# LIS-TU-Berlin/SVN-ICP

Hardware: AMD Instinct MI355X
Metric: scan-pair registrations/sec at N particles x M source pts, 1/2/4/8 GPU (higher is better)
Workload: dtype f64; 1 GPU; C3: 128 particles SVN-ICP, 131072-pt source vs 262144-pt target, K=100, I=20, max_dist=1.0, lr=1.0, SVNFullGrad=False, correspondence=fast, early stop off; synthetic 64-beam scans (seed 20250718); particles=128, target_points=262144, knn_count=100, parallelism=single GPU

## Files before the change

### include/svnicp_hip.h

```cpp
#ifndef SVNICP_HIP_H
#define SVNICP_HIP_H

#include <stdint.h>

#ifdef __cplusplus
extern "C" {
#endif

#define SVNICP_ABI_VERSION 1

typedef struct svnicp_ctx svnicp_ctx;

#define SVNICP_ALIGN_SUCCESS 1
#define SVNICP_NO_OPTIMIZER 2

typedef enum {
  SVNICP_OK = 0,
  SVNICP_ERR_INVALID = -1,
  SVNICP_ERR_HIP = -2,
  SVNICP_ERR_NO_DEVICE = -3,
  SVNICP_ERR_NOMEM = -4
} svnicp_status;

#define SVNICP_MODE_SVN 0
// ... 143 lines not shown
int svnicp_get_mode_labels(svnicp_ctx *ctx, int32_t *outP);

int svnicp_set_shard(svnicp_ctx *ctx, int p_lo, int p_hi);
int svnicp_set_row_shard(svnicp_ctx *ctx, int row_rank, int row_world, int64_t total_source_points);
void *svnicp_rank_sums_devptr(svnicp_ctx *ctx);
int svnicp_align_begin(svnicp_ctx *ctx);
int svnicp_stage_candidates(svnicp_ctx *ctx, int64_t b_lo, int64_t b_hi);
int svnicp_build_candidate_table(svnicp_ctx *ctx);
int svnicp_iter_accumulate(svnicp_ctx *ctx, int iteration);
int svnicp_iter_update(svnicp_ctx *ctx, int iteration);
int svnicp_finish(svnicp_ctx *ctx);
int svnicp_stopped(svnicp_ctx *ctx);
void *svnicp_candidates_devptr(svnicp_ctx *ctx);
void *svnicp_sums_devptr(svnicp_ctx *ctx);
void *svnicp_total_pose_devptr(svnicp_ctx *ctx);
#define SVNICP_NSUMS 22

typedef struct svnicp_map svnicp_map;
int svnicp_map_create(int device, double voxel_size, double max_range, int max_points, int64_t capacity_voxels,
                      svnicp_map **out);
void svnicp_map_destroy(svnicp_map *map);
const char *svnicp_map_last_error(const svnicp_map *map);
int svnicp_map_clear(svnicp_map *map);
int svnicp_map_size(svnicp_map *map, int64_t *voxels);
int svnicp_map_add_cloud(svnicp_map *map, const float *xyz, int64_t n, int mem_kind, const double R_rowmajor[9],
                         const double t[3]);
int svnicp_map_skipped_points(svnicp_map *map, int64_t *out);
int svnicp_map_table_info(svnicp_map *map, int64_t *capacity_slots, int64_t *tombstones, int64_t *rebuilds);
int svnicp_map_query(svnicp_map *map, const double center[3], double max_range, int64_t *count_out);
void *svnicp_map_points_devptr(svnicp_map *map);
// ... 92 lines not shown
```

### svn-icp_amd/binding.py

```python
from __future__ import annotations

import ctypes as C
import os
import re

_HERE = os.path.dirname(os.path.abspath(__file__))
_ROOT = os.path.dirname(_HERE)
_LIB_PATH = os.path.join(_HERE, "libsvnicp_hip.so")
_HEADER = os.path.join(_ROOT, "include", "svnicp_hip.h")


class SvnIcpError(RuntimeError):
    pass


class Params(C.Structure):
    _fields_ = [("struct_size", C.c_int32), ("mode", C.c_int32), ("iterations", C.c_int32),
                ("knn_count", C.c_int32), ("lr", C.c_double), ("max_dist", C.c_double),
                ("convergence_threshold", C.c_double), ("check_early_stop", C.c_int32),
                ("svn_full_grad", C.c_int32), ("optimizer", C.c_int32), ("record_trace", C.c_int32)]


class SegParamsStruct(C.Structure):
    _fields_ = [("struct_size", C.c_int32), ("n_scan", C.c_int32), ("horizon_scan", C.c_int32), ("ground_scan_ind", C.c_int32),
# ... 158 lines not shown
    L.svnicp_rank_sums_devptr.argtypes = [vp]
    L.svnicp_rank_sums_devptr.restype = vp
    L.svnicp_align_begin.argtypes = [vp]
    L.svnicp_stage_candidates.argtypes = [vp, C.c_int64, C.c_int64]
    L.svnicp_build_candidate_table.argtypes = [vp]
    L.svnicp_iter_accumulate.argtypes = [vp, C.c_int]
    L.svnicp_iter_update.argtypes = [vp, C.c_int]
    L.svnicp_finish.argtypes = [vp]
    L.svnicp_stopped.argtypes = [vp]
    L.svnicp_candidates_devptr.argtypes = [vp]
    L.svnicp_candidates_devptr.restype = vp
    L.svnicp_sums_devptr.argtypes = [vp]
    L.svnicp_sums_devptr.restype = vp
    L.svnicp_total_pose_devptr.argtypes = [vp]
    L.svnicp_total_pose_devptr.restype = vp
    L.svnicp_set_minibatch.argtypes = [vp, C.c_int, C.c_uint64]
    L.svnicp_set_minibatch_indices.argtypes = [vp, vp, C.c_int, C.c_int, C.c_int]
    L.svnicp_get_minibatch_indices.argtypes = [vp, ip]
    L.svnicp_get_minibatch_candidates.argtypes = [vp, ip]
    L.svnicp_get_minibatch_rows.argtypes = [vp, C.POINTER(C.c_int64)]
    L.svnicp_set_residual.argtypes = [vp, C.c_int, C.c_double, C.c_int]
    L.svnicp_set_target_normals.argtypes = [vp, vp, C.c_int64, C.c_int]
    L.svnicp_get_target_normals.argtypes = [vp, dp]
    L.svnicp_get_plane_stats.argtypes = [vp, dp, C.POINTER(C.c_int64)]
    L.svnicp_evaluate.argtypes = [vp, dp, dp, C.c_double, C.POINTER(EvalStruct)]
    for name in ("svnicp_eval_index_devptr", "svnicp_eval_dist2_devptr"):
        getattr(L, name).argtypes = [vp]
        getattr(L, name).restype = vp
    L.svnicp_get_eval_pairs.argtypes = [vp, ip, dp]
    L.svnicp_eval_information.argtypes = [vp, C.c_int, C.c_double, C.c_double, C.POINTER(InformationStruct)]
# ... 15 lines not shown
```

### svn-icp_amd/csrc/api.hip

```cpp
#include "../../include/svnicp_hip.h"

#include <cmath>
#include <algorithm>
#include <cstdio>
#include <cstdlib>
#include <cstring>
#include <string>
#include <vector>

#include "device_buffer.hpp"
#include "information_solve.hpp"
#include "kernels.hpp"
#include "stage_a_host.hpp"
#include "stage_b_host.hpp"

using namespace svnicp;
using namespace svnicp_host;

namespace {

struct CloudState {
  DevBuf<double> src, tgt;
  bool src_set = false, tgt_set = false;
};
// ... 400 lines not shown
  else if (k == "wgpcu") { int x = 0, y = 0; ok = sscanf(v.c_str(), "%d,%d", &x, &y) == 2 && x >= 0 && x <= 64 && y >= 0 && y <= 16; if (ok) { t.wgpcu_search = x; t.wgpcu_accum = y; } }
  else if (k == "tp") ok = num(0, 1 << 16, &t.tp);
  else if (k == "debug") ok = num(0, 1, &t.debug);
  else if (k == "scan_split") ok = num(0, 16, &t.scan_split);
  else if (k == "group_stride") ok = num(0, 1 << 30, &t.group_stride);
  else if (k == "accum_min_steps") ok = num(0, 1 << 20, &t.accum_min_steps);
  else if (k == "brute_qb") { ok = num(0, 6, &t.brute_qb); }
  else if (k == "single") { if (v == "fused") t.single_fused = 1; else if (v == "split") t.single_fused = 0; else ok = false; }
  else if (k == "chain") { if (v == "auto") { t.small_chain = 1; t.persistent = 0; } else if (v == "persistent") { t.small_chain = 1; t.persistent = 1; }
                           else if (v == "general") { t.small_chain = 0; t.persistent = 0; } else ok = false; }
  else if (k == "median") { if (v == "auto") t.median_inline = -1; else if (v == "stream") t.median_inline = 0; else if (v == "inline") t.median_inline = 1; else ok = false; }
  else if (k == "sort") { if (v == "joint") t.sort_joint = 1; else if (v == "separate") t.sort_joint = 0; else ok = false; }
  else if (k == "sort_kernel") { if (v == "radix") t.sort_merge = 0; else if (v == "merge") t.sort_merge = 1; else ok = false; }
  else if (k == "table") { if (v == "select") t.table_select = 1; else if (v == "gather") t.table_select = 0; else ok = false; }
  else if (k == "correspondence") { if (v == "fast") t.full_corr = 0; else if (v == "full") t.full_corr = 1; else ok = false; }
  else return fail(c, SVNICP_ERR_INVALID, "svnicp_set_option: unknown option '" + k + "'");
  if (!ok) return fail(c, SVNICP_ERR_INVALID, "svnicp_set_option: bad value '" + v + "' for option '" + k + "'");
  c->run.have_candidates = false;
  c->sa.held = TargetLayout::None;
  if (c->run.began) c->st.step = plan_step(registration_facts(c, c->pl.on), c->tune, c->sb.plan);
  return SVNICP_OK;
}

int svnicp_set_shard(svnicp_ctx* c, int p_lo, int p_hi) {
  CTX_CHECK(c);
  if (!c->run.particles_set || p_lo < 0 || p_hi > c->P || p_lo > p_hi)
    return fail(c, SVNICP_ERR_INVALID, "svnicp_set_shard: need 0 <= p_lo <= p_hi <= P after svnicp_set_particles");
  c->shard.p_lo = p_lo; c->shard.p_hi = p_hi; c->shard.set = true;
  return SVNICP_OK;
}
// ... 227 lines not shown
  }
  u.eul = c->st.eul.p; u.opt = c->st.opt.p; u.optimizer = c->prm.optimizer;
  u.n_src = (double)(c->shard.row_world > 1 ? c->shard.B_total : c->B);
  u.uctl = c->st.uctl.p;
  u.dbg = c->tune.debug ? c->dbg.upd.p : nullptr;
  u.svgd = c->prm.mode == SVNICP_MODE_SVGD ? 1 : 0;
  u.plane_Hb = c->pl.on ? c->pl.Hb.p : nullptr;
  return u;
}
static AccumArgs accum_args(svnicp_ctx* c, int it) {
  AccumArgs a{};
  a.src = c->cloud.src.p; a.table = c->sb.table.p; a.tablef = c->sb.tablef.p; a.tablea = c->sb.tablea.p; a.kbest = c->sb.kbest.p; a.kidx = c->sb.kidx.p; a.tgt = c->cloud.tgt.p; a.cand = c->sa.cand_idx.p; a.anchor = c->sb.anchor.p; a.M = c->M; a.cmax = c->sb.cmaxb.p; a.ambig_count = c->sb.ambig.p;
  a.Rtot = c->st.Rtot.p; a.B = c->B; a.K = c->K;
  a.p_lo = c->shard.p_lo; a.p_hi = c->shard.p_hi; a.max_dist = c->prm.max_dist; a.partial = c->sb.partial.p; a.ctl = c->st.ctl.p;
  a.corr = c->prm.record_trace ? c->tr.corr.p + (size_t)it * c->P * c->B : nullptr;
  if (c->mb.on) {
    const size_t r0 = (size_t)it * c->mb.batch;
    a.src = c->mb.src.p + 3 * r0; a.cand = c->mb.cand.p + r0 * c->K; a.cmax = c->sb.cmaxb.p + r0; a.B = c->mb.batch;
    if (c->sb.table.p) a.table = c->sb.table.p + r0 * c->K * 3;
    if (c->sb.tablef.p) a.tablef = c->sb.tablef.p + r0 * c->K;
    if (c->sb.tablea.p) a.tablea = c->sb.tablea.p + r0 * 128;
    if (c->sb.anchor.p) a.anchor = c->sb.anchor.p + 3 * r0;
    if (c->prm.record_trace) a.corr = c->tr.corr.p + (size_t)it * c->P * c->mb.batch;
  }
  a.svgd = c->prm.mode == SVNICP_MODE_SVGD ? 1 : 0;
  a.fin_iteration = -1;
  if (c->st.drive.defer_fin && it >= 1) {
    const UpdateArgs up = update_args(c, it - 1);
    a.fin_iteration = it - 1; a.fin_P = c->P; a.fin_thr = c->prm.convergence_threshold; a.fin_norms = update_step_norms(up);
    a.fin_pose = c->st.pose_out.p; a.fin_history = c->st.history.p; a.fin_ctl = c->st.ctl.p;
// ... 140 lines not shown
  return SVNICP_OK;
}

int svnicp_stopped(svnicp_ctx* c) {
  CTX_CHECK(c);
  if (bind(c)) return SVNICP_ERR_HIP;
  int v[2] = {0, 0};
  HIPCHK(c, hipMemcpyAsync(v, c->st.ctl.p, sizeof v, hipMemcpyDeviceToHost, c->stream));
  HIPCHK(c, hipStreamSynchronize(c->stream));
  return v[0] ? 1 : 0;
}

void* svnicp_candidates_devptr(svnicp_ctx* c) { return c ? (void*)c->sa.cand_idx.p : nullptr; }
void* svnicp_sums_devptr(svnicp_ctx* c) { return c ? (void*)c->sb.sums.p : nullptr; }
void* svnicp_total_pose_devptr(svnicp_ctx* c) { return c ? (void*)c->st.Rtot.p : nullptr; }

static int align_enqueue(svnicp_ctx* c, bool follow_stop) {
  CTX_CHECK(c);
  if (c->prm.mode == SVNICP_MODE_SVGD && (c->prm.optimizer < 0 || c->prm.optimizer > 3))
    return SVNICP_NO_OPTIMIZER;
  int rc = svnicp_align_begin(c);
  if (rc) return rc;
  if ((rc = svnicp_stage_candidates(c, 0, c->B))) return rc;
  if ((rc = svnicp_build_candidate_table(c))) return rc;
  c->st.small_launched = false;
  const DrivePlan drive = plan_drive(registration_facts(c, c->pl.on), c->tune, c->sb.plan, c->st.step, follow_stop);
  c->st.drive = drive;
  c->st.drive.defer_fin = false;
  if (drive.persistent_try) {
    const AccumArgs a = accum_args(c, 0);
// ... 595 lines not shown
```

### svn-icp_amd/csrc/kernels.hpp

```cpp
#pragma once
#include "device_math.hpp"
#include "registration_plan.hpp"
#include "stage_a_plan.hpp"

namespace svnicp {

struct KnnArgs {
  const double* src;
  Pose0 pose;
  const double *tx, *ty, *tz;
  const int32_t* torig;
  int64_t M, Mp;
  int64_t b_lo, b_hi;
  int K, S;
  double* pool_d;
  int32_t* pool_i;
  int32_t* out_idx;
  double* out_d2;
  const int32_t* qlist;
  const int* qlist_count;
  int list_grid;
  int list_qw;
  int slices, slice_max_queries, merge_n;
  double* sl_d;
// ... 104 lines not shown
  int p_lo, p_hi;
  int TP;
  int tiles_per_block;
  int64_t n_tiles;
  int Ppad;
  double max_dist;
  double* partial;
  const int* ctl;
  int32_t* corr;
  int svgd;
  const double* tgt;
  const int32_t* cand;
  const double* anchor;
  int64_t M;
  uint8_t* kbest;
  int32_t* kidx;
  const int32_t* full_idx;
  int pts_per_block, spts_per_block;
  unsigned int* ticket;
  int fin_iteration, fin_P;
  double fin_thr;
  const double* fin_norms;
  const double* fin_pose;
  float* fin_history;
  int* fin_ctl;
};
AccumPlan plan_accumulate(AccumPlan shape, int64_t B, int num_cus, const Tuning& tune);
hipError_t launch_search_split(const AccumPlan& plan, AccumArgs a, hipStream_t st);
hipError_t launch_accumulate_split(const AccumPlan& plan, const AccumArgs& a, hipStream_t st);
void split_occupancy_blocks(int PW, int WP, int K, size_t smem, int* search, int* accum);
// ... 171 lines not shown
```

### svn-icp_amd/csrc/registration_plan.hpp

```cpp
#pragma once
#include <cstddef>
#include <cstdint>
#include <initializer_list>

#include "stage_a_plan.hpp"

namespace svnicp {

struct Tuning {
  KnnOption knn;
  int knn_prefilter_mfma = 1;
  int fallback_sliced_max = -1;
  int accum = 3;
  int update_fused = 0;
  int fused_update_max_p = 128;
  int wgpcu_search = 0, wgpcu_accum = 0;
  int tp = 0;
  int accum_min_steps = 0;
  int group_stride = 0;
  int scan_split = 0;
  int debug = 0;
  int single_fused = 1;
  int small_chain = 1;
  int persistent = 0;
  int median_inline = -1;
  int brute_qb = 0;
  int sort_joint = 1;
  int sort_merge = 0;
  int table_select = 1;
  int full_corr = 0;
};

struct RegistrationFacts {
  int P = 0, K = 0, I = 0;
  int64_t B = 0, M = 0;
  bool svgd = false, check_early_stop = false, record_trace = false;
  bool profiling = false;
  bool shard_set = false;
  int p_lo = 0, p_hi = 0;
  int row_world = 1;
  int batch = 0;
  bool explicit_tab = false;
  int tab_I = 0;
  bool plane = false;
  bool normals_supplied = false;
// ... 166 lines not shown
```

### svn-icp_amd/csrc/search_limits.hpp

```cpp
#pragma once
#include <cstdint>

namespace svnicp {

constexpr int64_t kSearchPointsPerStep = 4;

constexpr int64_t search_offset_bound(int Ppad, int K) {
  return 4 * kSearchPointsPerStep * (int64_t)(Ppad > K ? Ppad : K);
}
constexpr bool search_offsets_fit(int Ppad, int K) { return search_offset_bound(Ppad, K) <= ((int64_t)1 << 32); }

}
```

### svn-icp_amd/csrc/small_registration.hip

```cpp
#include "kernels.hpp"
#include "stein_step_device.hpp"
#include "stein_split_device.hpp"

namespace svnicp {

namespace {

struct SmallArgs {
  int GS;
  int GA;
  int spts_per_block;
  int iterations;
  unsigned int* bar;
};

__device__ __forceinline__ bool grid_barrier(const SmallArgs& s, unsigned int& k, int nblocks, bool wait = true) {
  __shared__ int sh_ok;
  __syncthreads();
  if (threadIdx.x == 0) {
    int ok = 1;
    __threadfence();
    volatile unsigned int* vb = s.bar;
    unsigned int* cnt = s.bar + 4 + (k & 3u);
    if (atomicAdd(cnt, 1u) == (unsigned int)nblocks - 1u) {
// ... 3 lines not shown
    } else if (wait) {
      unsigned int polls = 0u;
      while ((int)(vb[0] - (k + 1u)) < 0) {
        __builtin_amdgcn_s_sleep(4);
        if (++polls > (1u << 22) || vb[1] != 0u) { atomicExch(&s.bar[1], 1u); ok = 0; break; }
      }
    }
    __threadfence();
    sh_ok = ok;
  }
  __syncthreads();
  ++k;
  return sh_ok != 0;
}

template <int PW, int WP, int NRB, bool TAIL, bool SVGD>
__global__ __launch_bounds__(256) void k_small_registration(AccumArgs a, UpdateArgs u, SmallArgs s) {
  extern __shared__ __align__(16) double dyn[];
  const int bx = (int)blockIdx.x, nblocks = (int)gridDim.x;
  const int P = u.P;
  const int n_prep = prepare_blocks(u), n_dir = direction_blocks(P);
  const bool want_finish = u.check_early_stop != 0;
  UpdateArgs ub = u;
  ub.sums = a.partial; ub.n_ranks = s.GA; ub.sums_stride = a.Ppad * kNSums;
  AccumArgs as = a;
  as.spts_per_block = s.spts_per_block;
  unsigned int k = 0u;
  PhaseStamp stamp(u.dbg, bx == 0 && threadIdx.x == 0);
  for (int it = 0; it < s.iterations; ++it) {
    if (a.ctl[0]) break;
    u.iteration = it; ub.iteration = it;
    if (bx < s.GS) search_body<PW, WP, NRB, TAIL>(as, bx, 0);
    stamp(0);
    if (bx == s.GS) {
      if (!grid_barrier(s, k, nblocks, false)) return;
      median_body<256>(u);
    } else {
      if (!grid_barrier(s, k, nblocks)) return;
      stamp(1);
      if (bx < s.GA) accumulate_body<PW, WP, true, SVGD>(a, bx, 0, dyn);
      stamp(2);
    }
    if (!grid_barrier(s, k, nblocks)) return;
    stamp(3);
    if (bx < n_prep) prepare_body(ub, bx);
    stamp(4);
    if (!grid_barrier(s, k, nblocks)) return;
// ... 2 lines not shown
    stamp(6);
    if (!grid_barrier(s, k, nblocks)) return;
    stamp(7);
    if (want_finish) {
      if (bx == 0) finish_body(u);
      if (!grid_barrier(s, k, nblocks)) return;
    }
  }
}

}

namespace {
template <int PW, int WP, int NRB, bool TAIL>
hipError_t launch_small_t(const AccumArgs& a, const UpdateArgs& u, const SmallArgs& s, int grid, size_t smem, hipStream_t st) {
  const void* fn = u.svgd ? reinterpret_cast<const void*>(k_small_registration<PW, WP, NRB, TAIL, true>)
                          : reinterpret_cast<const void*>(k_small_registration<PW, WP, NRB, TAIL, false>);
  hipError_t e = hipFuncSetAttribute(fn, hipFuncAttributeMaxDynamicSharedMemorySize, (int)smem);
  if (e != hipSuccess) return e;
  int per_cu = 0;
  e = hipOccupancyMaxActiveBlocksPerMultiprocessor(&per_cu, fn, 256, smem);
  if (e != hipSuccess) return e;
  if (per_cu < 1) return hipErrorCooperativeLaunchTooLarge;
  AccumArgs aa = a; UpdateArgs uu = u; SmallArgs ss = s;
  void* args[3] = {&aa, &uu, &ss};
  return hipLaunchCooperativeKernel(fn, dim3((unsigned)grid), dim3(256), args, (unsigned int)smem, st);
}
}

hipError_t launch_small_registration(const AccumPlan& plan, AccumArgs a, const UpdateArgs& u, int iterations, unsigned int* bar,
                                     int num_cus, hipStream_t st) {
  const int P = u.P;
// ... 28 lines not shown
```

### svn-icp_amd/csrc/stein_split.hip

```cpp
#include "stein_split_device.hpp"

namespace svnicp {

namespace {

__device__ __forceinline__ void build_table3_row(const int32_t* __restrict__ idx, int64_t b, int K, const double* __restrict__ tgt, int64_t M,
                                                 double* __restrict__ table, double* __restrict__ anchor, float4* __restrict__ tablea,
                                                 float* __restrict__ cmax, float* rb, int lane) {
  int64_t i0 = idx[b * K];
  i0 = i0 < 0 ? 0 : (i0 >= M ? M - 1 : i0);
  const double a0 = tgt[3 * i0], a1 = tgt[3 * i0 + 1], a2 = tgt[3 * i0 + 2];
  float cm = 0.0f;
  for (int k = lane; k < 128; k += kWave) {
    float4 row = table_sentinel_row();
    if (k < K) {
      int64_t i = idx[b * K + k];
      i = i < 0 ? 0 : (i >= M ? M - 1 : i);
      const double x = tgt[3 * i], y = tgt[3 * i + 1], z = tgt[3 * i + 2];
      if (table) {
        double* o = table + ((size_t)b * K + k) * 3;
        o[0] = x; o[1] = y; o[2] = z;
      }
      row = table_row(x, y, z, a0, a1, a2);
      cm = table_row_cmax(cm, row);
// ... 29 lines not shown
  const int lane = threadIdx.x & (kWave - 1), wave = threadIdx.x >> 6;
  const int64_t n = *count;
  for (int64_t e = (int64_t)blockIdx.x * 4 + wave; e < n && e < B; e += (int64_t)gridDim.x * 4) {
    const int64_t b = list[e];
    if (b < 0 || b >= B) continue;
    build_table3_row(idx, b, K, tgt, M, nullptr, anchor, tablea, cmax, rowbuf[wave], lane);
    __builtin_amdgcn_wave_barrier();
  }
}


inline int row_code_for(int K) { return K <= 16 ? 1 : K <= 32 ? 2 : K <= 64 ? 4 : K <= 96 ? 6 : K <= 100 ? 60 : K <= 112 ? 7 : 8; }

template <int PW, int WP, int NRB, bool TAIL>
hipError_t launch_s(const AccumPlan& plan, const AccumArgs& a, hipStream_t st) {
  hipLaunchKernelGGL((k_stein_search_bf16<PW, WP, NRB, TAIL>), dim3(plan.sgrid_x, plan.grid_y), dim3(NT), 0, st, a);
  return hipGetLastError();
}
template <int PW, int WP>
hipError_t launch_srb(const AccumPlan& plan, const AccumArgs& a, hipStream_t st) {
  switch (row_code_for(a.K)) {
    case 1: return launch_s<PW, WP, 1, false>(plan, a, st);
    case 2: return launch_s<PW, WP, 2, false>(plan, a, st);
    case 4: return launch_s<PW, WP, 4, false>(plan, a, st);
    case 6: return launch_s<PW, WP, 6, false>(plan, a, st);
    case 60: return launch_s<PW, WP, 6, true>(plan, a, st);
    case 7: return launch_s<PW, WP, 7, false>(plan, a, st);
    default: return launch_s<PW, WP, 8, false>(plan, a, st);
  }
}
template <int PW, int WP>
// ... 102 lines not shown
```

### svn-icp_amd/csrc/stein_split_device.hpp

```cpp
#pragma once
#include <cstdlib>
#include "kernels.hpp"
#include "stein_common.hpp"
#include "search_limits.hpp"

namespace svnicp {

namespace {

typedef float v4f __attribute__((ext_vector_type(4)));
#define SVNICP_CONST_AS __attribute__((address_space(4)))

__device__ __forceinline__ float pack_slot(float v, unsigned int mask, unsigned int bits) {
  return __uint_as_float((__float_as_uint(v) & ~mask) | bits);
}
__device__ __forceinline__ float imin_f(float a, float b) {
  const int x = (int)__float_as_uint(a), y = (int)__float_as_uint(b);
  return __uint_as_float((unsigned int)(x < y ? x : y));
}
__device__ __forceinline__ float imax_f(float a, float b) {
  const int x = (int)__float_as_uint(a), y = (int)__float_as_uint(b);
  return __uint_as_float((unsigned int)(x > y ? x : y));
}

// ... 103 lines not shown
    const int ok = __shfl_xor(bk, off, kWave);
    if (od < bd || (od == bd && ok < bk)) { bd = od; bk = ok; }
  }
  const double d0 = __shfl(d_first, (threadIdx.x & (kWave - 1)) & ~(G - 1), kWave);
  return (d0 != d0 || bk == 0x7fffffff) ? 0 : bk;
}

#ifndef SVNICP_SEARCH_EPS_U
#define SVNICP_SEARCH_EPS_U 54
#endif
constexpr float kEpsBf16 = (float)SVNICP_SEARCH_EPS_U * 5.9604644775390625e-08f;

#ifndef SVNICP_SEARCH_WAVES
#define SVNICP_SEARCH_WAVES 4
#endif
template <int PW, int WP, int NRB, bool TAIL>
__device__ __forceinline__ void search_body(const AccumArgs& a, int bx, int by) {
  if (a.ctl[0]) return;
  if (a.fin_iteration >= 0 && bx == 0 && by == 0) {
    __shared__ double sh_fin[NT];
    __shared__ int sh_fin_stop;
    const int ftid = threadIdx.x, FP = a.fin_P;
    double fs = 0.0;
    for (int p = ftid; p < FP; p += NT) fs += a.fin_norms[p];
    sh_fin[ftid] = fs;
    __syncthreads();
    for (int off = NT / 2; off > 0; off >>= 1) {
      if (ftid < off) sh_fin[ftid] += sh_fin[ftid + off];
      __syncthreads();
    }
    if (ftid == 0) {
      const double m = sh_fin[0] / FP;
      const int stop = (float)m < (float)a.fin_thr;
      if (stop) { a.fin_ctl[0] = 1; a.fin_ctl[1] = a.fin_iteration + 1; }
      sh_fin_stop = stop;
    }
    __syncthreads();
    if (sh_fin_stop) return;
    for (int e = ftid; e < 6 * FP; e += NT) a.fin_history[(size_t)a.fin_iteration * 6 * FP + e] = (float)a.fin_pose[e];
  }
  constexpr int BW = kWave / PW;
  constexpr int CBP = PW / 16;
  constexpr int NPT = 4 / CBP;
  constexpr int ST = 4 * BW;
  constexpr bool PIPE = NPT == 1;
  constexpr int NTILE = 4 * NRB + (TAIL ? 1 : 0);
  constexpr int RS = 16 * (((4 * NTILE + 15) / 16) | 1);
  __shared__ float4 s_rows[4][NPT][4][RS / 4];
  __shared__ float4 s_scr4[4][64];
  __shared__ double s_pose[WP][12][64];
  __shared__ unsigned int s_queue[kQueueCap];
  __shared__ unsigned int s_qn, s_qsteps;
  const int tid = threadIdx.x;
  if (tid == 0) { s_qn = 0u; s_qsteps = 0u; }
#pragma unroll
  for (int i = 0; i < kQueueCap / NT; ++i) s_queue[tid + i * NT] = 0xffffffffu;
  const int lane = tid & (kWave - 1);
  const int wave = __builtin_amdgcn_readfirstlane(tid >> 6);
  const int pl = lane % PW, bs = lane / PW;
  const int mj = lane & 15, mk = lane >> 4;
  const int pbase = by * (WP * PW);
  for (int g = wave; g < WP; g += 4) {
    const int p = a.p_lo + pbase + g * PW + pl;
    const double* rp = a.Rtot + 12 * (size_t)(p < a.p_hi ? p : a.p_lo);
#pragma unroll
    for (int i = 0; i < 12; ++i) s_pose[g][i][lane] = rp[i];
  }
  const int K = a.K;
  const SVNICP_CONST_AS v4f* ctab = (const SVNICP_CONST_AS v4f*)a.tablea;
  float* const rows_w = reinterpret_cast<float*>(&s_rows[wave][0][mk][0]) + mj;
  const int64_t blk_lo = (int64_t)bx * a.spts_per_block;
  const int64_t blk_hi = (blk_lo + a.spts_per_block < a.B) ? blk_lo + a.spts_per_block : a.B;
  static_assert(BW <= kSearchPointsPerStep, "search_limits.hpp bounds the pair offsets for at most this many points per step");
  __syncthreads();
  const int64_t nfirst = blk_lo + wave * BW;

  int pend_idx = 0;
  int32_t* pend_row = a.kidx;
  unsigned int pend_off4 = 0;
  bool pend_have = false;
  v4f alo_n, ahi_n;
  double sa_n = 0.0;
  float c_n = 0.0f;
  auto fetch_point = [&](int64_t nn) {
    const double* base = lane < 3 ? a.src + 3 * nn : a.anchor + 3 * nn - 3;
// ... 90 lines not shown

#pragma unroll
      for (int cb = 0; cb < 4; ++cb) {
        if constexpr (!PIPE) {
          if (cb % CBP == 0) {
            split_rows(ralo_n[cb / CBP], rahi_n[cb / CBP], cb / CBP);
            fetch_rows(n + ST, cb / CBP);
          }
        }
        const bf8 bfr = split_b3(braw[cb]);
        const v4f zero = {0.0f, 0.0f, 0.0f, 0.0f};
        float m1 = 0.0f, m2 = 0.0f, wp = 0.0f, rp = 0.0f, pend0 = 0.0f, pend1 = 0.0f;
        int np = 0;
        bool have_m = false;
        bool have_p = false;
        v4f dcur = __builtin_amdgcn_mfma_f32_16x16x32_bf16(afr[0], bfr, zero, 0, 0, 0);
        v4f dnext = dcur;
        if (NRB > 1) dnext = __builtin_amdgcn_mfma_f32_16x16x32_bf16(afr[NRB > 1 ? 1 : 0], bfr, zero, 0, 0, 0);
#pragma unroll
        for (int rb = 0; rb < NRB; ++rb) {
          v4f dn2 = dnext;
          if (rb + 2 < NRB) dn2 = __builtin_amdgcn_mfma_f32_16x16x32_bf16(afr[rb + 2 < NRB ? rb + 2 : 0], bfr, zero, 0, 0, 0);
          const float pk = pack_slot3(fmin_raw(fmin3_raw(dcur[0], dcur[1], dcur[2]), dcur[3]), 4u * rb);
          if (np == 0) { pend0 = pk; np = 1; }
          else if (np == 1) { pend1 = pk; np = 2; }
          else {
            np = 0;
            const float w = fmin3_raw(pend0, pend1, pk), r = fmed3_raw(pend0, pend1, pk);
            if (!have_p) { wp = w; rp = r; have_p = true; }
            else {
              have_p = false;
              if (!have_m) {
                m1 = fmin_raw(wp, w);
                m2 = fmin3_raw(fmax_raw(wp, w), rp, r);
                have_m = true;
              } else {
                const float md = fmed3_raw(m1, wp, w);
                m2 = fmin_raw(fmin3_raw(m2, rp, r), md);
                m1 = fmin3_raw(m1, wp, w);
              }
            }
          }
          dcur = dnext; dnext = dn2;
        }
        if (!have_m) { m1 = __builtin_huge_valf(); m2 = __builtin_huge_valf(); }
        if (have_p) { const float t = fmax_raw(m1, wp); m1 = fmin_raw(m1, wp); m2 = fmin3_raw(t, m2, rp); }
        if (np >= 1) { m2 = fmed3_raw(m1, m2, pend0); m1 = fmin_raw(m1, pend0); }
        if (np >= 2) { m2 = fmed3_raw(m1, m2, pend1); m1 = fmin_raw(m1, pend1); }
        b1[cb] = m1; b2[cb] = m2;
      }
#pragma unroll
      for (int cb = 0; cb < 4; ++cb) b1[cb] = __uint_as_float(__builtin_amdgcn_bitop3_b32(__float_as_uint(b1[cb]), 3u, (unsigned int)mk, 0xBA));
      auto merge2 = [&](float p1, float q1, float p2, float q2, float& o1, float& o2) {
        o1 = fmin_raw(p1, q1);
        o2 = fmin_raw(fmax_raw(p1, q1), fmin_raw(p2, q2));
      };
      float b1own, b2own;
      {
        float h1[2], h2[2];
#pragma unroll
        for (int j = 0; j < 2; ++j) {
          const auto r1 = __builtin_amdgcn_permlane16_swap(__float_as_uint(b1[2 * j]), __float_as_uint(b1[2 * j + 1]), false, false);
          const auto r2 = __builtin_amdgcn_permlane16_swap(__float_as_uint(b2[2 * j]), __float_as_uint(b2[2 * j + 1]), false, false);
          merge2(__uint_as_float(r1[0]), __uint_as_float(r1[1]), __uint_as_float(r2[0]), __uint_as_float(r2[1]), h1[j], h2[j]);
        }
        const auto r1 = __builtin_amdgcn_permlane32_swap(__float_as_uint(h1[0]), __float_as_uint(h1[1]), false, false);
        const auto r2 = __builtin_amdgcn_permlane32_swap(__float_as_uint(h2[0]), __float_as_uint(h2[1]), false, false);
        merge2(__uint_as_float(r1[0]), __uint_as_float(r1[1]), __uint_as_float(r2[0]), __uint_as_float(r2[1]), b1own, b2own);
      }
      auto score_tile = [&](int tile, float* sc) {
        const float4 cx = s_rows[wave][bs][0][tile], cy = s_rows[wave][bs][1][tile];
        const float4 cz = s_rows[wave][bs][2][tile], cc = s_rows[wave][bs][3][tile];
        sc[0] = __builtin_fmaf(cx.x, mm0, __builtin_fmaf(cy.x, mm1, __builtin_fmaf(cz.x, mm2, cc.x)));
        sc[1] = __builtin_fmaf(cx.y, mm0, __builtin_fmaf(cy.y, mm1, __builtin_fmaf(cz.y, mm2, cc.y)));
        sc[2] = __builtin_fmaf(cx.z, mm0, __builtin_fmaf(cy.z, mm1, __builtin_fmaf(cz.z, mm2, cc.z)));
        sc[3] = __builtin_fmaf(cx.w, mm0, __builtin_fmaf(cy.w, mm1, __builtin_fmaf(cz.w, mm2, cc.w)));
      };
      if constexpr (TAIL) {
        float sc[4];
        score_tile(4 * NRB, sc);
        const float pk = pack_slot3(fmin_raw(fmin3_raw(sc[0], sc[1], sc[2]), sc[3]), 4u * NRB);
        b2own = fmed3_raw(b1own, b2own, pk);
        b1own = fmin_raw(b1own, pk);
      }

      const int pin = g * PW + pl;
      const bool valid = inb && (a.p_lo + pbase + pin) < a.p_hi;
      int tile = (int)(__float_as_uint(b1own) & 31u);
      tile = tile < NTILE ? tile : NTILE - 1;
      const float thr = 2.0f * E + 3.83e-06f * (__builtin_fabsf(b1own) + __builtin_fabsf(b2own)) + 1.0e-30f;
      const bool tiles_ok = b2own - b1own > thr;
      float pk4[4];
      {
        if constexpr (!PIPE) __builtin_amdgcn_wave_barrier();
        float sc[4];
        score_tile(tile, sc);
#pragma unroll
        for (int t = 0; t < 4; ++t) pk4[t] = __uint_as_float(__builtin_amdgcn_bitop3_b32(__float_as_uint(sc[t]), 3u, (unsigned int)t, 0xBA));
      }
      const float w3 = fmin3_raw(pk4[0], pk4[1], pk4[2]), r3 = fmed3_raw(pk4[0], pk4[1], pk4[2]);
      const float v1 = fmin_raw(w3, pk4[3]), v2 = fmed3_raw(w3, r3, pk4[3]);
      const float thrv = 2.0f * E + 4.76837158203125e-07f * (__builtin_fabsf(v1) + __builtin_fabsf(v2)) + 1.0e-30f;
      int kb = 4 * tile + (int)(__float_as_uint(v1) & 3u);
      const bool ambiguous = valid & (!tiles_ok | !(v2 - v1 > thrv) | (kb >= K));
      kb = kb < K ? kb : K - 1;
      unsigned long long am = __ballot(ambiguous);
      if (am) {
        const int cnt = __builtin_popcountll(am);
        int base = 0;
        if (lane == 0) { base = (int)atomicAdd(&s_qn, (unsigned int)cnt); atomicAdd(&s_qsteps, 1u); }
        base = __builtin_amdgcn_readfirstlane(base);
        if (base + cnt <= kQueueCap) {
          if (ambiguous) {
            const int rank = __builtin_popcountll(am & ((1ull << lane) - 1ull));
            s_queue[base + rank] = ((unsigned int)(b - blk_lo) << 8) | (unsigned int)pin;
          }
        } else {
          do {
            const int L = (int)__builtin_ctzll(am);
            am &= am - 1;
            const int ke = exact_nearest_of_k<kWave>(a, s_pose[g], n + L / PW, L % PW, K, lane);
            if (lane == L) kb = ke;
          } while (am);
        }
      }
      if (pend_have) *(int32_t*)((char*)pend_row + pend_off4) = pend_idx;
      pend_have = inb;
      pend_row = a.kidx + n * a.Ppad + pbase;
      if (inb) {
        const unsigned int bl = (unsigned int)bs;
        const unsigned int off = bl * (unsigned int)a.Ppad + (unsigned int)pin;
        (a.kbest + n * a.Ppad + pbase)[off] = (uint8_t)kb;
        pend_off4 = 4u * off;
        pend_idx = *(const int32_t*)((const char*)(a.cand + n * K) + 4u * (bl * (unsigned int)K + (unsigned int)kb));
      }
    }
    __builtin_amdgcn_wave_barrier();
  }

  if (pend_have) *(int32_t*)((char*)pend_row + pend_off4) = pend_idx;
  __syncthreads();
  {
    const unsigned int total = s_qn < (unsigned int)kQueueCap ? s_qn : (unsigned int)kQueueCap;
    constexpr int kExactLanes = 32;
    const int sub = lane & (kExactLanes - 1);
    for (unsigned int e = (unsigned int)(tid / kExactLanes); e < total; e += NT / kExactLanes) {
      const unsigned int ent = s_queue[e];
      if (ent == 0xffffffffu) continue;
      const int64_t be = blk_lo + (int64_t)(ent >> 8);
      const int pin = (int)(ent & 0xffu);
      const int ke = exact_nearest_of_k<kExactLanes>(a, s_pose[pin / PW], be, pin % PW, K, sub);
      if (sub == 0) {
        a.kbest[(size_t)be * a.Ppad + (pbase + pin)] = (uint8_t)ke;
        a.kidx[(size_t)be * a.Ppad + (pbase + pin)] = a.cand[(size_t)be * K + ke];
      }
    }
    if (tid == 0 && a.ambig_count && s_qsteps) { atomicAdd(a.ambig_count, (int)s_qsteps); atomicAdd(a.ambig_count + 1, (int)s_qn); }
  }
}

template <int PW, int WP, int NRB, bool TAIL>
__global__ __launch_bounds__(NT, (PW == 16 || WP == 4) ? 3 : SVNICP_SEARCH_WAVES) void k_stein_search_bf16(AccumArgs a) {
  search_body<PW, WP, NRB, TAIL>(a, xcd_block((int)blockIdx.x, (int)gridDim.x), (int)blockIdx.y);
}

template <int PW, int WP, bool PLAIN, bool SVGD = false>
__device__ __forceinline__ void accumulate_body(const AccumArgs& a, int bx, int by, double* lds) {
  if (a.ctl[0]) return;
  constexpr int BW = kWave / PW;
  constexpr int WB = 4 / WP;
#ifndef SVNICP_ACCUM_U
#define SVNICP_ACCUM_U 4
#endif
  constexpr int U = SVNICP_ACCUM_U;
  const int tid = threadIdx.x;
  const int lane = tid & (kWave - 1);
  const int wave = __builtin_amdgcn_readfirstlane(tid >> 6);
  const int wp = wave % WP, wb = wave / WP;
// ... 148 lines not shown
```

Before: 151.2 registrations/s.

## Add opt-in two-quad search tiles and skip winner-slot stores unless tracing

Adds an alternate search kernel variant that reduces candidate scores over tiles of two quads (eight candidates), selectable through a new search_tile option. It also skips writing the per-pair kbest byte unless trace recording is on, removing a scattered global store from the search hot loop. The two-quad path is off by default, so only the skipped kbest store runs with default settings. The risk is that code reading kbest outside trace mode now sees stale data.

```diff
diff --git a/include/svnicp_hip.h b/include/svnicp_hip.h
--- a/include/svnicp_hip.h
+++ b/include/svnicp_hip.h
@@ -181,6 +181,7 @@
 void *svnicp_candidates_devptr(svnicp_ctx *ctx);
 void *svnicp_sums_devptr(svnicp_ctx *ctx);
 void *svnicp_total_pose_devptr(svnicp_ctx *ctx);
+void *svnicp_winner_slot_devptr(svnicp_ctx *ctx);
 #define SVNICP_NSUMS 22
 
 typedef struct svnicp_map svnicp_map;
diff --git a/svn-icp_amd/binding.py b/svn-icp_amd/binding.py
--- a/svn-icp_amd/binding.py
+++ b/svn-icp_amd/binding.py
@@ -196,6 +196,8 @@
     L.svnicp_sums_devptr.restype = vp
     L.svnicp_total_pose_devptr.argtypes = [vp]
     L.svnicp_total_pose_devptr.restype = vp
+    L.svnicp_winner_slot_devptr.argtypes = [vp]
+    L.svnicp_winner_slot_devptr.restype = vp
     L.svnicp_set_minibatch.argtypes = [vp, C.c_int, C.c_uint64]
     L.svnicp_set_minibatch_indices.argtypes = [vp, vp, C.c_int, C.c_int, C.c_int]
     L.svnicp_get_minibatch_indices.argtypes = [vp, ip]
diff --git a/svn-icp_amd/csrc/api.hip b/svn-icp_amd/csrc/api.hip
--- a/svn-icp_amd/csrc/api.hip
+++ b/svn-icp_amd/csrc/api.hip
@@ -438,6 +438,7 @@
   else if (k == "sort_kernel") { if (v == "radix") t.sort_merge = 0; else if (v == "merge") t.sort_merge = 1; else ok = false; }
   else if (k == "table") { if (v == "select") t.table_select = 1; else if (v == "gather") t.table_select = 0; else ok = false; }
   else if (k == "correspondence") { if (v == "fast") t.full_corr = 0; else if (v == "full") t.full_corr = 1; else ok = false; }
+  else if (k == "search_tile") { if (v == "4") t.search_tile = 4; else if (v == "8") t.search_tile = 8; else ok = false; }
   else return fail(c, SVNICP_ERR_INVALID, "svnicp_set_option: unknown option '" + k + "'");
   if (!ok) return fail(c, SVNICP_ERR_INVALID, "svnicp_set_option: bad value '" + v + "' for option '" + k + "'");
   c->run.have_candidates = false;
@@ -695,6 +696,8 @@
   a.Rtot = c->st.Rtot.p; a.B = c->B; a.K = c->K;
   a.p_lo = c->shard.p_lo; a.p_hi = c->shard.p_hi; a.max_dist = c->prm.max_dist; a.partial = c->sb.partial.p; a.ctl = c->st.ctl.p;
   a.corr = c->prm.record_trace ? c->tr.corr.p + (size_t)it * c->P * c->B : nullptr;
+  a.store_kbest = c->prm.record_trace ? 1 : 0;
+  a.search_tile = c->tune.search_tile;
   if (c->mb.on) {
     const size_t r0 = (size_t)it * c->mb.batch;
     a.src = c->mb.src.p + 3 * r0; a.cand = c->mb.cand.p + r0 * c->K; a.cmax = c->sb.cmaxb.p + r0; a.B = c->mb.batch;
@@ -865,6 +868,7 @@
 void* svnicp_candidates_devptr(svnicp_ctx* c) { return c ? (void*)c->sa.cand_idx.p : nullptr; }
 void* svnicp_sums_devptr(svnicp_ctx* c) { return c ? (void*)c->sb.sums.p : nullptr; }
 void* svnicp_total_pose_devptr(svnicp_ctx* c) { return c ? (void*)c->st.Rtot.p : nullptr; }
+void* svnicp_winner_slot_devptr(svnicp_ctx* c) { return c ? (void*)c->sb.kbest.p : nullptr; }
 
 static int align_enqueue(svnicp_ctx* c, bool follow_stop) {
   CTX_CHECK(c);
diff --git a/svn-icp_amd/csrc/kernels.hpp b/svn-icp_amd/csrc/kernels.hpp
--- a/svn-icp_amd/csrc/kernels.hpp
+++ b/svn-icp_amd/csrc/kernels.hpp
@@ -142,6 +142,8 @@
   const double* anchor;
   int64_t M;
   uint8_t* kbest;
+  int store_kbest;
+  int search_tile;
   int32_t* kidx;
   const int32_t* full_idx;
   int pts_per_block, spts_per_block;
diff --git a/svn-icp_amd/csrc/registration_plan.hpp b/svn-icp_amd/csrc/registration_plan.hpp
--- a/svn-icp_amd/csrc/registration_plan.hpp
+++ b/svn-icp_amd/csrc/registration_plan.hpp
@@ -29,6 +29,7 @@
   int sort_merge = 0;
   int table_select = 1;
   int full_corr = 0;
+  int search_tile = 0;
 };
 
 struct RegistrationFacts {
diff --git a/svn-icp_amd/csrc/search_limits.hpp b/svn-icp_amd/csrc/search_limits.hpp
--- a/svn-icp_amd/csrc/search_limits.hpp
+++ b/svn-icp_amd/csrc/search_limits.hpp
@@ -10,4 +10,7 @@
 }
 constexpr bool search_offsets_fit(int Ppad, int K) { return search_offset_bound(Ppad, K) <= ((int64_t)1 << 32); }
 
+constexpr int search_default_quads(int PW) { return 1; }
+constexpr bool search_runs_alt(int PW, int search_tile) { return search_tile != 0 && search_tile != 4 * search_default_quads(PW); }
+
 }
diff --git a/svn-icp_amd/csrc/small_registration.hip b/svn-icp_amd/csrc/small_registration.hip
--- a/svn-icp_amd/csrc/small_registration.hip
+++ b/svn-icp_amd/csrc/small_registration.hip
@@ -41,7 +41,7 @@
   return sh_ok != 0;
 }
 
-template <int PW, int WP, int NRB, bool TAIL, bool SVGD>
+template <int PW, int WP, int NRB, bool TAIL, bool SVGD, int TQ>
 __global__ __launch_bounds__(256) void k_small_registration(AccumArgs a, UpdateArgs u, SmallArgs s) {
   extern __shared__ __align__(16) double dyn[];
   const int bx = (int)blockIdx.x, nblocks = (int)gridDim.x;
@@ -57,7 +57,7 @@
   for (int it = 0; it < s.iterations; ++it) {
     if (a.ctl[0]) break;
     u.iteration = it; ub.iteration = it;
-    if (bx < s.GS) search_body<PW, WP, NRB, TAIL>(as, bx, 0);
+    if (bx < s.GS) search_body<PW, WP, NRB, TAIL, TQ>(as, bx, 0);
     stamp(0);
     if (bx == s.GS) {
       if (!grid_barrier(s, k, nblocks, false)) return;
@@ -90,8 +90,12 @@
 namespace {
 template <int PW, int WP, int NRB, bool TAIL>
 hipError_t launch_small_t(const AccumArgs& a, const UpdateArgs& u, const SmallArgs& s, int grid, size_t smem, hipStream_t st) {
-  const void* fn = u.svgd ? reinterpret_cast<const void*>(k_small_registration<PW, WP, NRB, TAIL, true>)
-                          : reinterpret_cast<const void*>(k_small_registration<PW, WP, NRB, TAIL, false>);
+  constexpr int TD = search_default_quads(PW);
+  const bool alt = search_runs_alt(PW, a.search_tile);
+  const void* fn = u.svgd ? (alt ? reinterpret_cast<const void*>(k_small_registration<PW, WP, NRB, TAIL, true, 3 - TD>)
+                                 : reinterpret_cast<const void*>(k_small_registration<PW, WP, NRB, TAIL, true, TD>))
+                          : (alt ? reinterpret_cast<const void*>(k_small_registration<PW, WP, NRB, TAIL, false, 3 - TD>)
+                                 : reinterpret_cast<const void*>(k_small_registration<PW, WP, NRB, TAIL, false, TD>));
   hipError_t e = hipFuncSetAttribute(fn, hipFuncAttributeMaxDynamicSharedMemorySize, (int)smem);
   if (e != hipSuccess) return e;
   int per_cu = 0;
diff --git a/svn-icp_amd/csrc/stein_split.hip b/svn-icp_amd/csrc/stein_split.hip
--- a/svn-icp_amd/csrc/stein_split.hip
+++ b/svn-icp_amd/csrc/stein_split.hip
@@ -67,7 +67,8 @@
 
 template <int PW, int WP, int NRB, bool TAIL>
 hipError_t launch_s(const AccumPlan& plan, const AccumArgs& a, hipStream_t st) {
-  hipLaunchKernelGGL((k_stein_search_bf16<PW, WP, NRB, TAIL>), dim3(plan.sgrid_x, plan.grid_y), dim3(NT), 0, st, a);
+  if (search_runs_alt(PW, a.search_tile)) hipLaunchKernelGGL((k_stein_search_bf16_alt<PW, WP, NRB, TAIL>), dim3(plan.sgrid_x, plan.grid_y), dim3(NT), 0, st, a);
+  else hipLaunchKernelGGL((k_stein_search_bf16<PW, WP, NRB, TAIL>), dim3(plan.sgrid_x, plan.grid_y), dim3(NT), 0, st, a);
   return hipGetLastError();
 }
 template <int PW, int WP>
diff --git a/svn-icp_amd/csrc/stein_split_device.hpp b/svn-icp_amd/csrc/stein_split_device.hpp
--- a/svn-icp_amd/csrc/stein_split_device.hpp
+++ b/svn-icp_amd/csrc/stein_split_device.hpp
@@ -141,8 +141,10 @@
 #ifndef SVNICP_SEARCH_WAVES
 #define SVNICP_SEARCH_WAVES 4
 #endif
-template <int PW, int WP, int NRB, bool TAIL>
+template <int PW, int WP, int NRB, bool TAIL, int TQ>
 __device__ __forceinline__ void search_body(const AccumArgs& a, int bx, int by) {
+  static_assert(TQ == 1 || TQ == 2, "tiles of one or two quads");
+  static_assert(TQ == 1 || !TAIL || NRB % 2 == 0, "the tail quad's index 4·NRB is 8·(pair count) only behind whole pairs");
   if (a.ctl[0]) return;
   if (a.fin_iteration >= 0 && bx == 0 && by == 0) {
     __shared__ double sh_fin[NT];
@@ -171,8 +173,11 @@
   constexpr int NPT = 4 / CBP;
   constexpr int ST = 4 * BW;
   constexpr bool PIPE = NPT == 1;
-  constexpr int NTILE = 4 * NRB + (TAIL ? 1 : 0);
-  constexpr int RS = 16 * (((4 * NTILE + 15) / 16) | 1);
+  constexpr int NQ = 4 * NRB + (TAIL ? 1 : 0);
+  constexpr int NPR = (NRB + 1) / 2;
+  constexpr int NTILE = TQ == 1 ? NQ : 4 * NPR + (TAIL ? 1 : 0);
+  constexpr bool PADQ = TQ == 2 && (TAIL || NRB % 2 == 1);
+  constexpr int RS = 16 * (((4 * (NQ + (PADQ ? 4 : 0)) + 15) / 16) | 1);
   __shared__ float4 s_rows[4][NPT][4][RS / 4];
   __shared__ float4 s_scr4[4][64];
   __shared__ double s_pose[WP][12][64];
@@ -194,8 +199,13 @@
     for (int i = 0; i < 12; ++i) s_pose[g][i][lane] = rp[i];
   }
   const int K = a.K;
+  const bool store_kb = a.store_kbest != 0;
   const SVNICP_CONST_AS v4f* ctab = (const SVNICP_CONST_AS v4f*)a.tablea;
   float* const rows_w = reinterpret_cast<float*>(&s_rows[wave][0][mk][0]) + mj;
+  if constexpr (PADQ) {
+#pragma unroll
+    for (int pt = 0; pt < NPT; ++pt) rows_w[pt * 4 * RS + 4 * NQ] = mk == 3 ? kSentinelCC : 0.0f;
+  }
   const int64_t blk_lo = (int64_t)bx * a.spts_per_block;
   const int64_t blk_hi = (blk_lo + a.spts_per_block < a.B) ? blk_lo + a.spts_per_block : a.B;
   static_assert(BW <= kSearchPointsPerStep, "search_limits.hpp bounds the pair offsets for at most this many points per step");
@@ -316,6 +326,7 @@
         int np = 0;
         bool have_m = false;
         bool have_p = false;
+        float tmin[NPR];
         v4f dcur = __builtin_amdgcn_mfma_f32_16x16x32_bf16(afr[0], bfr, zero, 0, 0, 0);
         v4f dnext = dcur;
         if (NRB > 1) dnext = __builtin_amdgcn_mfma_f32_16x16x32_bf16(afr[NRB > 1 ? 1 : 0], bfr, zero, 0, 0, 0);
@@ -323,6 +334,16 @@
         for (int rb = 0; rb < NRB; ++rb) {
           v4f dn2 = dnext;
           if (rb + 2 < NRB) dn2 = __builtin_amdgcn_mfma_f32_16x16x32_bf16(afr[rb + 2 < NRB ? rb + 2 : 0], bfr, zero, 0, 0, 0);
+          if constexpr (TQ == 2) {
+            if (rb % 2 == 0) {
+              pend0 = fmin_raw(fmin3_raw(dcur[0], dcur[1], dcur[2]), dcur[3]);
+              if (rb == NRB - 1) tmin[rb / 2] = pack_slot3(pend0, 4u * (rb / 2));
+            } else {
+              tmin[rb / 2] = pack_slot3(fmin3_raw(fmin3_raw(pend0, dcur[0], dcur[1]), dcur[2], dcur[3]), 4u * (rb / 2));
+            }
+            dcur = dnext; dnext = dn2;
+            continue;
+          }
           const float pk = pack_slot3(fmin_raw(fmin3_raw(dcur[0], dcur[1], dcur[2]), dcur[3]), 4u * rb);
           if (np == 0) { pend0 = pk; np = 1; }
           else if (np == 1) { pend1 = pk; np = 2; }
@@ -345,10 +366,19 @@
           }
           dcur = dnext; dnext = dn2;
         }
-        if (!have_m) { m1 = __builtin_huge_valf(); m2 = __builtin_huge_valf(); }
-        if (have_p) { const float t = fmax_raw(m1, wp); m1 = fmin_raw(m1, wp); m2 = fmin3_raw(t, m2, rp); }
-        if (np >= 1) { m2 = fmed3_raw(m1, m2, pend0); m1 = fmin_raw(m1, pend0); }
-        if (np >= 2) { m2 = fmed3_raw(m1, m2, pend1); m1 = fmin_raw(m1, pend1); }
+        if constexpr (TQ == 2) {
+          if constexpr (NPR == 1) { m1 = tmin[0]; m2 = __builtin_huge_valf(); }
+          else if constexpr (NPR == 2) { m1 = fmin_raw(tmin[0], tmin[1]); m2 = fmax_raw(tmin[0], tmin[1]); }
+          else {
+            m1 = fmin3_raw(tmin[0], tmin[1], tmin[2]); m2 = fmed3_raw(tmin[0], tmin[1], tmin[2]);
+            if constexpr (NPR == 4) { m2 = fmed3_raw(m1, m2, tmin[3]); m1 = fmin_raw(m1, tmin[3]); }
+          }
+        } else {
+          if (!have_m) { m1 = __builtin_huge_valf(); m2 = __builtin_huge_valf(); }
+          if (have_p) { const float t = fmax_raw(m1, wp); m1 = fmin_raw(m1, wp); m2 = fmin3_raw(t, m2, rp); }
+          if (np >= 1) { m2 = fmed3_raw(m1, m2, pend0); m1 = fmin_raw(m1, pend0); }
+          if (np >= 2) { m2 = fmed3_raw(m1, m2, pend1); m1 = fmin_raw(m1, pend1); }
+        }
         b1[cb] = m1; b2[cb] = m2;
       }
 #pragma unroll
@@ -370,9 +400,9 @@
         const auto r2 = __builtin_amdgcn_permlane32_swap(__float_as_uint(h2[0]), __float_as_uint(h2[1]), false, false);
         merge2(__uint_as_float(r1[0]), __uint_as_float(r1[1]), __uint_as_float(r2[0]), __uint_as_float(r2[1]), b1own, b2own);
       }
-      auto score_tile = [&](int tile, float* sc) {
-        const float4 cx = s_rows[wave][bs][0][tile], cy = s_rows[wave][bs][1][tile];
-        const float4 cz = s_rows[wave][bs][2][tile], cc = s_rows[wave][bs][3][tile];
+      auto score_tile = [&](int quad, float* sc) {
+        const float4 cx = s_rows[wave][bs][0][quad], cy = s_rows[wave][bs][1][quad];
+        const float4 cz = s_rows[wave][bs][2][quad], cc = s_rows[wave][bs][3][quad];
         sc[0] = __builtin_fmaf(cx.x, mm0, __builtin_fmaf(cy.x, mm1, __builtin_fmaf(cz.x, mm2, cc.x)));
         sc[1] = __builtin_fmaf(cx.y, mm0, __builtin_fmaf(cy.y, mm1, __builtin_fmaf(cz.y, mm2, cc.y)));
         sc[2] = __builtin_fmaf(cx.z, mm0, __builtin_fmaf(cy.z, mm1, __builtin_fmaf(cz.z, mm2, cc.z)));
@@ -381,7 +411,7 @@
       if constexpr (TAIL) {
         float sc[4];
         score_tile(4 * NRB, sc);
-        const float pk = pack_slot3(fmin_raw(fmin3_raw(sc[0], sc[1], sc[2]), sc[3]), 4u * NRB);
+        const float pk = pack_slot3(fmin_raw(fmin3_raw(sc[0], sc[1], sc[2]), sc[3]), TQ == 1 ? 4u * NRB : 4u * NPR);
         b2own = fmed3_raw(b1own, b2own, pk);
         b1own = fmin_raw(b1own, pk);
       }
@@ -392,18 +422,39 @@
       tile = tile < NTILE ? tile : NTILE - 1;
       const float thr = 2.0f * E + 3.83e-06f * (__builtin_fabsf(b1own) + __builtin_fabsf(b2own)) + 1.0e-30f;
       const bool tiles_ok = b2own - b1own > thr;
-      float pk4[4];
-      {
-        if constexpr (!PIPE) __builtin_amdgcn_wave_barrier();
-        float sc[4];
-        score_tile(tile, sc);
-#pragma unroll
-        for (int t = 0; t < 4; ++t) pk4[t] = __uint_as_float(__builtin_amdgcn_bitop3_b32(__float_as_uint(sc[t]), 3u, (unsigned int)t, 0xBA));
-      }
-      const float w3 = fmin3_raw(pk4[0], pk4[1], pk4[2]), r3 = fmed3_raw(pk4[0], pk4[1], pk4[2]);
-      const float v1 = fmin_raw(w3, pk4[3]), v2 = fmed3_raw(w3, r3, pk4[3]);
-      const float thrv = 2.0f * E + 4.76837158203125e-07f * (__builtin_fabsf(v1) + __builtin_fabsf(v2)) + 1.0e-30f;
-      int kb = 4 * tile + (int)(__float_as_uint(v1) & 3u);
+      float v1, v2;
+      int kb;
+      if constexpr (!PIPE) __builtin_amdgcn_wave_barrier();
+      if constexpr (TQ == 1) {
+        float pk4[4];
+        {
+          float sc[4];
+          score_tile(tile, sc);
+#pragma unroll
+          for (int t = 0; t < 4; ++t) pk4[t] = __uint_as_float(__builtin_amdgcn_bitop3_b32(__float_as_uint(sc[t]), 3u, (unsigned int)t, 0xBA));
+        }
+        const float w3 = fmin3_raw(pk4[0], pk4[1], pk4[2]), r3 = fmed3_raw(pk4[0], pk4[1], pk4[2]);
+        v1 = fmin_raw(w3, pk4[3]); v2 = fmed3_raw(w3, r3, pk4[3]);
+        kb = 4 * tile + (int)(__float_as_uint(v1) & 3u);
+      } else {
+        const int qa = tile + 4 * (tile >> 2);
+        float pk8[8];
+        {
+          float sc[8];
+          score_tile(qa, sc);
+          score_tile(qa + 4, sc + 4);
+#pragma unroll
+          for (int t = 0; t < 8; ++t) pk8[t] = __uint_as_float(__builtin_amdgcn_bitop3_b32(__float_as_uint(sc[t]), 7u, (unsigned int)t, 0xBA));
+        }
+        const float wa = fmin3_raw(pk8[0], pk8[1], pk8[2]), ra = fmed3_raw(pk8[0], pk8[1], pk8[2]);
+        const float wb = fmin3_raw(pk8[3], pk8[4], pk8[5]), rb3 = fmed3_raw(pk8[3], pk8[4], pk8[5]);
+        const float wc = fmin_raw(pk8[6], pk8[7]), rc = fmax_raw(pk8[6], pk8[7]);
+        v2 = fmin_raw(fmin3_raw(ra, rb3, rc), fmed3_raw(wa, wb, wc));
+        v1 = fmin3_raw(wa, wb, wc);
+        const unsigned int vb = __float_as_uint(v1);
+        kb = (int)(((vb & 4u) << 2) | (4u * (unsigned int)qa + (vb & 3u)));
+      }
+      const float thrv = 2.0f * E + (TQ == 1 ? 4.76837158203125e-07f : 9.5367431640625e-07f) * (__builtin_fabsf(v1) + __builtin_fabsf(v2)) + 1.0e-30f;
       const bool ambiguous = valid & (!tiles_ok | !(v2 - v1 > thrv) | (kb >= K));
       kb = kb < K ? kb : K - 1;
       unsigned long long am = __ballot(ambiguous);
@@ -432,7 +483,7 @@
       if (inb) {
         const unsigned int bl = (unsigned int)bs;
         const unsigned int off = bl * (unsigned int)a.Ppad + (unsigned int)pin;
-        (a.kbest + n * a.Ppad + pbase)[off] = (uint8_t)kb;
+        if (store_kb) (a.kbest + n * a.Ppad + pbase)[off] = (uint8_t)kb;
         pend_off4 = 4u * off;
         pend_idx = *(const int32_t*)((const char*)(a.cand + n * K) + 4u * (bl * (unsigned int)K + (unsigned int)kb));
       }
@@ -453,7 +504,7 @@
       const int pin = (int)(ent & 0xffu);
       const int ke = exact_nearest_of_k<kExactLanes>(a, s_pose[pin / PW], be, pin % PW, K, sub);
       if (sub == 0) {
-        a.kbest[(size_t)be * a.Ppad + (pbase + pin)] = (uint8_t)ke;
+        if (store_kb) a.kbest[(size_t)be * a.Ppad + (pbase + pin)] = (uint8_t)ke;
         a.kidx[(size_t)be * a.Ppad + (pbase + pin)] = a.cand[(size_t)be * K + ke];
       }
     }
@@ -463,7 +514,11 @@
 
 template <int PW, int WP, int NRB, bool TAIL>
 __global__ __launch_bounds__(NT, (PW == 16 || WP == 4) ? 3 : SVNICP_SEARCH_WAVES) void k_stein_search_bf16(AccumArgs a) {
-  search_body<PW, WP, NRB, TAIL>(a, xcd_block((int)blockIdx.x, (int)gridDim.x), (int)blockIdx.y);
+  search_body<PW, WP, NRB, TAIL, search_default_quads(PW)>(a, xcd_block((int)blockIdx.x, (int)gridDim.x), (int)blockIdx.y);
+}
+template <int PW, int WP, int NRB, bool TAIL>
+__global__ __launch_bounds__(NT, (PW == 16 || WP == 4) ? 3 : SVNICP_SEARCH_WAVES) void k_stein_search_bf16_alt(AccumArgs a) {
+  search_body<PW, WP, NRB, TAIL, 3 - search_default_quads(PW)>(a, xcd_block((int)blockIdx.x, (int)gridDim.x), (int)blockIdx.y);
 }
 
 template <int PW, int WP, bool PLAIN, bool SVGD = false>
```

Result: no change. 152.7 registrations/s (median of 6 runs) (+1.0%).
